# Todegal/HobbyRaytracer

Measured on AMD Instinct MI355X. Metric: Mrays/sec (path segments/s), teapot_scene.yaml 640x640 100spp, higher is better.
Workload: dtype f32

## Files before the change

hobbyraytracer_amd/csrc/hrt_hip.hip:

```cpp
#include <hip/hip_runtime.h>
#include <rccl/rccl.h>
#include <dlfcn.h>

#include <algorithm>
#include <cmath>
#include <cstdio>
#include <cstdlib>
#include <cstring>
#include <memory>
#include <new>
#include <string>
#include <thread>
#include <type_traits>
#include <vector>

#include "hrt_device.h"
#include "hrt_pack.h"
#include "hrt_roulette.h"
#include "hrt_aov.h"
#include "hrt_map.h"

using namespace hrt;

namespace {
// ... 1102 lines not shown
        local += weight(i);
        out[i + 1] = ok ? (float)((s_run[t] + local) / total) : 0.0f;
    }
    __syncthreads();
    if (t == 0) { out[0] = 0.0f; out[n] = 1.0f; }
    return total;
}
__global__ __launch_bounds__(256) void k_env_rows(const float* __restrict__ texels, int W, int H, int channels, float* __restrict__ cond,
                                                  double* __restrict__ row_total) {
    __shared__ double s_run[257];
    const int j = blockIdx.x;
    double phi0, dphi, c0, dc;
    env_cell_bounds<double>(0, j, W, H, phi0, dphi, c0, dc);
    const float* row = texels + (size_t)j * (size_t)W * (size_t)channels;
    const double total = env_block_cdf(W, [&](int i) { return env_texel_weight(row + (size_t)i * (size_t)channels, i, W, dc); },
                                       cond + (size_t)j * (size_t)(W + 1), s_run);
    if (threadIdx.x == 0) row_total[j] = total;
}
__global__ __launch_bounds__(256) void k_env_marginal(const double* __restrict__ row_total, int H, float* __restrict__ marg, double* __restrict__ total) {
    __shared__ double s_run[257];
    const double t = env_block_cdf(H, [&](int j) { return row_total[j]; }, marg, s_run);
    if (threadIdx.x == 0) total[0] = t;
}

#define HRT_TAIL_MAX_MESHES 4
struct TailMeshes { int n; int prim[HRT_TAIL_MAX_MESHES]; };
template <bool STATS, int DEPTH>
__global__ __launch_bounds__(256, DEPTH <= 24 ? 4 : 3) void k_wf_tail(DScene sc, hrt_params pr, RenderMap map, WfScene ws, TailMeshes tm, unsigned n_local, int s0, int round0,
                                                    int rounds_end, WfBuf w, DeviceCounters* counters, int leaf_num) {
    const unsigned lane = threadIdx.x & 63u;
    const unsigned wave = (blockIdx.x * blockDim.x + threadIdx.x) >> 6;
    const unsigned long long lt = (1ull << lane) - 1ull;
    __shared__ int s_stack[DEPTH * 256];
    constexpr uint32_t TABLE_BYTES = DEPTH <= 20 ? 4096 : (DEPTH <= 24 ? 1536 : 4096);
    __shared__ __attribute__((aligned(16))) uint32_t s_tables[TABLE_BYTES / 4];
    __shared__ float s_missq[4][7 * HRT_MISSQ_CAP];
    stage_tables(sc, s_tables, TABLE_BYTES);
    MissQueue mq;
    mq.f = s_missq[threadIdx.x >> 6]; mq.slot = (unsigned*)(mq.f + 6 * HRT_MISSQ_CAP); mq.count = 0;
    unsigned n_seg = 0, n_culled = 0;
    PathCounters pc; pc.rays = 0; pc.samples = 0; pc.mesh_hits = 0; pc.env_lookups = 0; pc.bvh.box_tests = 0; pc.bvh.tri_tests = 0;
    DCounters cnt; cnt.box_tests = 0; cnt.tri_tests = 0;
    HRT_FOR_MY_TASKS(task, w, wave, lane) {
        unsigned live = HRT_UNIFORM(w.live[task]), qn = HRT_UNIFORM(w.qn[task]), rn = HRT_UNIFORM(w.rn[task]);
        for (int r = round0; r < rounds_end && live; ++r) {
            const int par = r & 1;
            for (int m = 0; m < tm.n; ++m) {
                if (m > 0) {
                    qn = wf_pre_task<STATS>(sc, pr, map, n_local, s0, r, par, tm.prim[m - 1] + 1, tm.prim[m], w, task, live, lane, lt, n_culled, rn);
                    __builtin_amdgcn_fence(__ATOMIC_ACQ_REL, "workgroup");
                }
                if (rn) {
                    wf_ref_task<STATS>(wf_ref_mesh(sc, tm.prim[m], pr.quirks), pr, tm.prim[m], par, w, task, rn, s_stack + (threadIdx.x & ~63u), DEPTH * 64u, lane, cnt);
                    __builtin_amdgcn_fence(__ATOMIC_ACQ_REL, "workgroup");
                }
                if (qn) {
                    const ExtMesh em = wf_ext_mesh(sc, tm.prim[m], pr.quirks);
                    bool given = false;
                    const unsigned first0 = task * w.T, end0 = first0 + qn;
                    wf_ext_run<STATS>(em, pr, tm.prim[m], par, w, s_stack + threadIdx.x, lane, lt, leaf_num, cnt, [&](unsigned& first, unsigned& end) {
                        if (given) return false;
                        given = true; first = first0; end = end0;
                        return true;
                    });
                    __builtin_amdgcn_fence(__ATOMIC_ACQ_REL, "workgroup");
                }
            }
            wf_shade_task<STATS>(sc, pr, map, ws, n_local, s0, r, w, task, live, lane, lt, mq, pc, n_seg, n_culled, live, qn, rn);
            __builtin_amdgcn_fence(__ATOMIC_ACQ_REL, "workgroup");
        }
        if (lane == 0) { w.live[task] = live; w.qn[task] = qn; w.rn[task] = rn; }
    }
    if (mq.count) missq_flush<STATS>(sc, w, mq, lane, mq.count, pc);
    wf_shade_counters<STATS>(w, counters, wave, lane, n_seg, n_culled, pc);
    if (STATS) {
        const unsigned bt = wave_sum(cnt.box_tests), tt = wave_sum(cnt.tri_tests);
        if (lane == 0) {
            if (bt) atomicAdd(&counters->box_tests, (unsigned long long)bt);
            if (tt) atomicAdd(&counters->tri_tests, (unsigned long long)tt);
        }
    }
}

__device__ inline float4 wf_sample_value(const float4* __restrict__ rad, const float4* __restrict__ direct, size_t i, bool nee) {
    float4 r = rad[i];
    if (nee) { const float4 d = direct[i]; r.x = r.x + d.x; r.y = r.y + d.y; r.z = r.z + d.z; }
    return r;
}
__device__ inline void wf_fold_shadow(DeviceCounters* counters, unsigned long long* __restrict__ wave_shadow, unsigned n_wave_rays) {
    __shared__ unsigned long long total_s;
    if (threadIdx.x == 0) total_s = 0;
    __syncthreads();
    unsigned long long mine = 0;
    for (unsigned i = threadIdx.x; i < n_wave_rays; i += blockDim.x) { mine += wave_shadow[i]; wave_shadow[i] = 0; }
    if (mine) atomicAdd(&total_s, mine);
    __syncthreads();
    if (threadIdx.x == 0 && total_s) atomicAdd(&counters->shadow_rays, total_s);
}
template <bool NEE>
__global__ __launch_bounds__(256) void k_wf_reduce(const float4* __restrict__ rad, unsigned n_local, int chunk, int first_chunk, int last_chunk,
                                                   int spp, float* __restrict__ out, DeviceCounters* counters,
                                                   unsigned long long* __restrict__ wave_rays, unsigned n_wave_rays,
                                                   const float4* __restrict__ direct, unsigned long long* __restrict__ wave_shadow) {
    const unsigned stride = gridDim.x * blockDim.x;
    for (unsigned lp = blockIdx.x * blockDim.x + threadIdx.x; lp < n_local; lp += stride) {
        vec3 sum(0.0f);
        if (!first_chunk) sum = vec3(out[3ull * lp], out[3ull * lp + 1], out[3ull * lp + 2]);
        for (int s = 0; s < chunk; ++s) {
            const float4 r = wf_sample_value(rad, direct, (size_t)s * n_local + lp, NEE);
            sum += vec3(r.x, r.y, r.z);
        }
        if (last_chunk) sum = sum / static_cast<float>(spp);
        out[3ull * lp] = sum.x; out[3ull * lp + 1] = sum.y; out[3ull * lp + 2] = sum.z;
    }
    if (blockIdx.x == 0) {
        __shared__ unsigned long long total;
        if (threadIdx.x == 0) total = 0;
        __syncthreads();
        unsigned long long mine = 0;
        for (unsigned i = threadIdx.x; i < n_wave_rays; i += blockDim.x) { mine += wave_rays[i]; wave_rays[i] = 0; }
        if (mine) atomicAdd(&total, mine);
        __syncthreads();
        if (threadIdx.x == 0) {
            if (total) atomicAdd(&counters->rays, total);
            atomicAdd(&counters->samples, (unsigned long long)n_local * (unsigned long long)chunk);
        }
        if (NEE) wf_fold_shadow(counters, wave_shadow, n_wave_rays);
    }
}

__global__ __launch_bounds__(256) void k_wf_progress(const unsigned* __restrict__ live, unsigned n_tasks, unsigned long long base_plus_slots,
                                                     volatile unsigned long long* host_ctr) {
    __shared__ unsigned long long total;
    if (threadIdx.x == 0) total = 0;
    __syncthreads();
    unsigned long long mine = 0;
    for (unsigned i = threadIdx.x; i < n_tasks; i += blockDim.x) mine += live[i];
    if (mine) atomicAdd(&total, mine);
    __syncthreads();
    if (threadIdx.x == 0) { *host_ctr = base_plus_slots - total; __threadfence_system(); }
}
__global__ void k_set_progress(unsigned long long v, volatile unsigned long long* host_ctr) { *host_ctr = v; __threadfence_system(); }

__global__ __launch_bounds__(256) void k_unstripe(const float* __restrict__ gathered, float* __restrict__ film, int H, int W3, int R, int G, long long share) {
    const long long n = (long long)H * W3;
    for (long long i = (long long)blockIdx.x * blockDim.x + threadIdx.x; i < n; i += (long long)gridDim.x * blockDim.x) {
        const int row = (int)(i / W3), x = (int)(i - (long long)row * W3);
        const int b = row / R, g = b % G, local = (b / G) * R + (row - b * R);
        film[i] = gathered[(long long)g * share + (long long)local * W3 + x];
    }
}
__global__ __launch_bounds__(256) void k_restripe(const float* __restrict__ film, float* __restrict__ mine, int H, int W3, int R, int G, int rank, int rows) {
    const long long n = (long long)rows * W3;
    for (long long i = (long long)blockIdx.x * blockDim.x + threadIdx.x; i < n; i += (long long)gridDim.x * blockDim.x) {
        const int local = (int)(i / W3), x = (int)(i - (long long)local * W3);
        const int b = local / R, row = (b * G + rank) * R + (local - b * R);
        mine[i] = film[(long long)row * W3 + x];
    }
}
__global__ __launch_bounds__(256) void k_preview_mean(const float* __restrict__ sums, float* __restrict__ mean, long long n, float samples_done) {
    for (long long i = (long long)blockIdx.x * blockDim.x + threadIdx.x; i < n; i += (long long)gridDim.x * blockDim.x) mean[i] = sums[i] / samples_done;
}



__device__ inline float ad_luma(float r, float g, float b) { return 0.2126f * r + 0.7152f * g + 0.0722f * b; }
// ... 85 lines not shown
        const unsigned v = i < n ? blocks[i] : 0u;
        part[threadIdx.x] = v;
        __syncthreads();
        for (unsigned off = 1; off < 256; off <<= 1) {
            const unsigned t = threadIdx.x >= off ? part[threadIdx.x - off] : 0u;
            __syncthreads();
            part[threadIdx.x] += t;
            __syncthreads();
        }
        if (i < n) blocks[i] = carry + part[threadIdx.x] - v;
        carry += part[255];
        __syncthreads();
    }
    if (threadIdx.x == 0) blocks[n] = carry;
}
__global__ __launch_bounds__(256) void k_ad_mean(const float* __restrict__ sums, const int32_t* __restrict__ count, long long n,
                                                 float* __restrict__ mean) {
    for (long long i = (long long)blockIdx.x * blockDim.x + threadIdx.x; i < n; i += (long long)gridDim.x * blockDim.x) {
        const float c = static_cast<float>(count[i]);
        mean[3 * i] = sums[3 * i] / c; mean[3 * i + 1] = sums[3 * i + 1] / c; mean[3 * i + 2] = sums[3 * i + 2] / c;
    }
}

}

namespace {
thread_local std::string g_err;

hrt_status fail_hip(hipError_t e, const char* what) {
    g_err = std::string(what) + ": " + hipGetErrorString(e);
    return HRT_ERR_HIP;
}
hrt_status fail(hrt_status s, const std::string& msg) { g_err = msg; return s; }
}
extern "C" __attribute__((visibility("hidden"))) void hrt_set_last_error(const char* msg) { g_err = msg; }
namespace {

#define HIPCHK(expr)                                         \
    do {                                                     \
        hipError_t _e = (expr);                              \
        if (_e != hipSuccess) return fail_hip(_e, #expr);    \
    } while (0)
#define HRTCHK(expr)                                         \
    do {                                                     \
        hrt_status _s = (expr);                              \
        if (_s != HRT_OK) return _s;                         \
    } while (0)

class DevBuf {
public:
    DevBuf() = default;
    DevBuf(DevBuf&& o) noexcept : p_(o.p_) { o.p_ = nullptr; }
    DevBuf& operator=(DevBuf&& o) noexcept { if (this != &o) { reset(); p_ = o.p_; o.p_ = nullptr; } return *this; }
    DevBuf(const DevBuf&) = delete;
    DevBuf& operator=(const DevBuf&) = delete;
    ~DevBuf() { reset(); }
    hrt_status alloc(size_t bytes, const char* what) {
        reset();
        hipError_t e = hipMalloc(&p_, bytes);
        if (e == hipSuccess) return HRT_OK;
        p_ = nullptr;
        return fail(e == hipErrorOutOfMemory ? HRT_ERR_OOM : HRT_ERR_HIP, std::string(what) + ": " + hipGetErrorString(e));
    }
    void reset() { if (p_) (void)hipFree(p_); p_ = nullptr; }
    template <typename T = void> T* get() const { return static_cast<T*>(p_); }
    explicit operator bool() const { return p_ != nullptr; }
private:
    void* p_ = nullptr;
};

hrt_status upload(DevBuf& buf, const void* src, size_t bytes) {
    HRTCHK(buf.alloc(bytes ? bytes : 16, "hipMalloc"));
    if (bytes) HIPCHK(hipMemcpy(buf.get(), src, bytes, hipMemcpyHostToDevice));
    return HRT_OK;
}

bool finite3(const float* p) { return p[0] == p[0] && p[1] == p[1] && p[2] == p[2]; }
}

struct WfWorkspace {
    DevBuf base;
    size_t bytes = 0;
    size_t slots = 0;
    int depth = 0, n_mesh = 0;
    bool nee = false;
    bool lobes = false;
    WfBuf buf{};
};

struct hrt_scene {
    int device = 0;
    int n_cus = 256;
    DScene ds{};
    std::vector<DevBuf> allocs;
    std::vector<int> mesh_prims;
    std::vector<int> mesh_depths;
    int n_prims = 0;
    DeviceCounters* d_counters = nullptr;
    unsigned* d_work = nullptr;
    WfWorkspace wf;
    struct Pending { hipEvent_t a, b; };
    std::vector<Pending> pending, pending_trav;
    std::vector<hipEvent_t> event_pool;
    double kernel_ms = 0.0, traversal_ms = 0.0;
    uint64_t launches = 0, traversal_launches = 0;
    volatile unsigned long long* h_progress = nullptr;
    unsigned long long* d_progress = nullptr;
    unsigned long long progress_base = 0;
    volatile unsigned long long progress_total = 0;
    DevBuf ad_pix, ad_blocks;
    size_t ad_cap = 0;
    float4* d_lights = nullptr;
    int32_t* d_light_of = nullptr;
    int n_lights = 0;
    DevBuf env_marg, env_cond;
    int env_w = 0, env_h = 0;
    DevBuf emit_rec, emit_shade, emit_alias, emit_base;
    int n_emit = 0;
    int32_t rr_first = HRT_ROULETTE_FIRST_BOUNCE;
    float rr_floor = HRT_ROULETTE_Q_FLOOR;
};

namespace {

hrt_status validate(const hrt_flat_scene* f) {
    if (!f) return fail(HRT_ERR_INVALID, "flat scene is NULL");
    if (f->n_prims && !f->prims) return fail(HRT_ERR_INVALID, "prims is NULL");
    if (f->n_textures == 0 || !f->textures) return fail(HRT_ERR_INVALID, "scene needs at least the background texture");
    if (f->background_tex < 0 || (uint32_t)f->background_tex >= f->n_textures) return fail(HRT_ERR_INVALID, "background_tex out of range");
    for (uint32_t i = 0; i < f->n_textures; ++i) {
        const hrt_texture& t = f->textures[i];
        if (t.kind < HRT_TEX_SOLID || t.kind > HRT_TEX_ENV) return fail(HRT_ERR_INVALID, "texture kind out of range");
        if (t.kind == HRT_TEX_CHECKER) {
            if (t.even < 0 || (uint32_t)t.even >= f->n_textures || t.odd < 0 || (uint32_t)t.odd >= f->n_textures)
                return fail(HRT_ERR_INVALID, "checker child out of range");
        }
        if (t.kind == HRT_TEX_IMAGE || t.kind == HRT_TEX_ENV) {
            if (t.width < 0 || t.height < 0) return fail(HRT_ERR_INVALID, "negative texture size");
            if (t.width > 0 && t.height > 0) {
                const bool env = t.kind == HRT_TEX_ENV;
                if (env && t.channels < 3) return fail(HRT_ERR_INVALID, "environment map needs >= 3 channels");
                const uint64_t have = env ? f->n_texels_f32 : f->n_texels_u8;
                const uint64_t per = (uint64_t)t.width * (uint64_t)t.height;
                const uint64_t ch = env ? (uint64_t)t.channels : 3u;
                if (t.offset > have || per > (have - t.offset) / ch) return fail(HRT_ERR_INVALID, env ? "env texels out of range" : "image texels out of range");
                if (have && !(env ? (const void*)f->texels_f32 : (const void*)f->texels_u8)) return fail(HRT_ERR_INVALID, "texel array is NULL");
            }
        }
    }
    for (uint32_t i = 0; i < f->n_textures; ++i) {
        if (f->textures[i].kind != HRT_TEX_CHECKER) continue;
        std::vector<std::pair<uint32_t, int>> st;
        st.push_back({i, 1});
        while (!st.empty()) {
            auto [t, depth] = st.back(); st.pop_back();
            if (f->textures[t].kind != HRT_TEX_CHECKER) continue;
            if (depth > 4) return fail(HRT_ERR_UNSUPPORTED, "checkered textures nested more than 4 deep (or cyclic)");
            st.push_back({(uint32_t)f->textures[t].even, depth + 1});
            st.push_back({(uint32_t)f->textures[t].odd, depth + 1});
        }
    }
    if (f->n_materials && !f->materials) return fail(HRT_ERR_INVALID, "materials is NULL");
    if (f->n_meshes && !f->meshes) return fail(HRT_ERR_INVALID, "meshes is NULL");
    if (f->n_nodes && !f->nodes) return fail(HRT_ERR_INVALID, "nodes is NULL");
    auto tex_ok = [&](int32_t t) { return t < 0 || (uint32_t)t < f->n_textures; };
    for (uint32_t i = 0; i < f->n_materials; ++i) {
        const hrt_material& m = f->materials[i];
// ... 139 lines not shown
    if ((int64_t)p->width * p->height > (int64_t)1 << 30) return fail(HRT_ERR_UNSUPPORTED, "film larger than 2^30 pixels");
    if (((int64_t)p->width + 7) / 8 * (((int64_t)p->height + 7) / 8) * 64 > (int64_t)0x7fffffff) return fail(HRT_ERR_UNSUPPORTED, "film too thin: its 8x8-tile padding exceeds 2^31 pixels");
    if (p->samples < 1) return fail(HRT_ERR_INVALID, "samples must be >= 1");
    if (p->max_depth < 1) return fail(HRT_ERR_INVALID, "max_depth must be >= 1");
    if (p->max_depth > 65536) return fail(HRT_ERR_UNSUPPORTED, "max_depth above 65536 (the reference's is 50, main.cpp:32)");
    if (!(p->t_min == p->t_min)) return fail(HRT_ERR_INVALID, "t_min is NaN");
    if ((p->flags & HRT_FLAG_NEE_ENV) && !(p->flags & HRT_FLAG_NEE)) return fail(HRT_ERR_INVALID, "HRT_FLAG_NEE_ENV needs HRT_FLAG_NEE");
    if ((p->flags & HRT_FLAG_NEE_EMITTERS) && !(p->flags & HRT_FLAG_NEE)) return fail(HRT_ERR_INVALID, "HRT_FLAG_NEE_EMITTERS needs HRT_FLAG_NEE");
    if ((p->flags & HRT_FLAG_NEE_LOBES) && !(p->flags & HRT_FLAG_NEE)) return fail(HRT_ERR_INVALID, "HRT_FLAG_NEE_LOBES needs HRT_FLAG_NEE");
    if ((p->flags & HRT_FLAG_MEGAKERNEL) && (p->flags & HRT_FLAG_NEE)) return fail(HRT_ERR_UNSUPPORTED, "next-event estimation renders on the wavefront pipeline only");
    if ((p->flags & HRT_FLAG_MEGAKERNEL) && (p->flags & HRT_FLAG_STRATIFIED)) return fail(HRT_ERR_UNSUPPORTED, "the stratified sampler renders on the wavefront pipeline only");
    if ((p->flags & HRT_FLAG_MEGAKERNEL) && (p->flags & HRT_FLAG_ROULETTE)) return fail(HRT_ERR_UNSUPPORTED, "Russian roulette renders on the wavefront pipeline only");
    if ((p->flags & HRT_FLAG_STATS) && (p->flags & HRT_FLAG_ROULETTE)) return fail(HRT_ERR_UNSUPPORTED, "HRT_FLAG_ROULETTE has no counting kernels (HRT_FLAG_STATS); rays and shadow_rays are counted without them");
    return HRT_OK;
}

hrt_status env_table_device(const float* d_texels, int W, int H, int channels, float* d_marg, float* d_cond, bool* has) {
    DevBuf d_rows, d_total;
    HRTCHK(d_rows.alloc((size_t)H * sizeof(double), "hipMalloc(env table)"));
    HRTCHK(d_total.alloc(sizeof(double), "hipMalloc(env table)"));
    hipLaunchKernelGGL(k_env_rows, dim3((unsigned)H), dim3(256), 0, 0, d_texels, W, H, channels, d_cond, d_rows.get<double>());
    hipLaunchKernelGGL(k_env_marginal, dim3(1), dim3(256), 0, 0, d_rows.get<const double>(), H, d_marg, d_total.get<double>());
    HIPCHK(hipGetLastError());
    double total = 0.0;
    HIPCHK(hipMemcpy(&total, d_total.get(), sizeof(double), hipMemcpyDeviceToHost));
    *has = total > 0.0 && std::isfinite(total);
    return HRT_OK;
}

hrt_status check_stripes(int32_t R, int32_t rank, int32_t G) {
    if (R <= 0 || G <= 0 || rank < 0 || rank >= G) return fail(HRT_ERR_INVALID, "bad stripe partition");
    return HRT_OK;
}

int grid_for(const hrt_scene* sc, long long n) { return (int)std::min<long long>((n + 255) / 256, (long long)sc->n_cus * 8); }

template <typename F>
void with_bool(bool b, F&& f) {
    if (b) f(std::true_type{});
    else f(std::false_type{});
}

int depth_variant(int depth) { return depth <= 20 ? 20 : (depth <= 24 ? 24 : 32); }
template <typename F>
void with_depth(int variant, F&& f) {
    switch (variant) {
        case 20: f(std::integral_constant<int, 20>{}); break;
        case 24: f(std::integral_constant<int, 24>{}); break;
        default: f(std::integral_constant<int, 32>{}); break;
    }
}

hrt_status get_event(hrt_scene* sc, hipEvent_t* ev) {
    if (!sc->event_pool.empty()) { *ev = sc->event_pool.back(); sc->event_pool.pop_back(); return HRT_OK; }
    HIPCHK(hipEventCreate(ev));
    return HRT_OK;
}

hrt_status launch_megakernel(hrt_scene* sc, const hrt_camera* cam, const hrt_params* pr, const RenderMap& map, float* d_out,
                             hipStream_t stream) {
    HIPCHK(hipMemsetAsync(sc->d_work, 0, sizeof(unsigned), stream));
    const int blocks = grid_for(sc, map.total_items);
    with_bool(pr->flags & HRT_FLAG_STATS, [&](auto S) {
        hipLaunchKernelGGL(k_pathtrace<decltype(S)::value>, dim3(blocks), dim3(HRT_BLOCK), 0, stream, sc->ds, *cam, *pr, map, d_out, sc->d_counters, sc->d_work);
    });
    HIPCHK(hipGetLastError());
    return HRT_OK;
}

size_t wf_max_slots(const hrt_scene* sc, bool nee = false, bool lobes = false) {
    if (const char* e = getenv("HRT_WF_MAX_SLOTS")) { long long v = atoll(e); if (v > 0) return (size_t)v; }
    size_t cap = (size_t)48 << 20;
    size_t free_b = 0, total_b = 0;
    if (hipMemGetInfo(&free_b, &total_b) == hipSuccess) {
        free_b += sc->wf.bytes;
        cap = std::max(cap, (size_t)((double)free_b * 0.6 / (lobes ? 264.0 : (nee ? 232.0 : 184.0))));
    }
    return std::min(cap, (size_t)1 << 31);
}

size_t wf_counter_words(int depth, int n_mesh) { return (size_t)256 * (2 + (size_t)depth * (2 * (size_t)std::max(1, n_mesh) + 2)); }
size_t wf_ref_counter_words(int depth, int n_mesh) { return (size_t)512 * ((size_t)depth * (size_t)std::max(1, n_mesh) + 1); }

hrt_status wf_reserve(hrt_scene* sc, size_t slots, int depth, bool nee, bool lobes) {
    WfWorkspace& w = sc->wf;
    const int n_mesh = (int)sc->mesh_prims.size();
    if (w.base && w.slots >= slots && w.depth >= depth && w.n_mesh == n_mesh && (w.nee || !nee) && (w.lobes || !lobes)) return HRT_OK;
    if (w.base) { HIPCHK(hipDeviceSynchronize()); w = WfWorkspace(); }
    const size_t max_tasks = slots / 64 + 1;
    auto al = [](size_t x) { return (x + 255) & ~(size_t)255; };
    const size_t f4 = al((slots + 4096) * sizeof(float4));
    const size_t i4 = al((slots + 4096) * sizeof(int));
    const size_t ctr_words = wf_counter_words(depth, n_mesh) + wf_ref_counter_words(depth, n_mesh);
    const size_t ref_cap = max_tasks / HRT_REF_GROUPS + 1;
    const size_t total = (sc->ds.stale_ff ? 12 : 11) * f4 + 2 * i4 + 3 * al(max_tasks * sizeof(unsigned)) + al(ctr_words * sizeof(unsigned)) + al(ref_cap * HRT_REF_GROUPS * sizeof(uint2)) +
                         al((size_t)sc->n_cus * 32 * sizeof(unsigned long long)) +
                         (nee ? 3 * f4 + al((size_t)sc->n_cus * 32 * sizeof(unsigned long long)) : 0) +
                         (lobes ? 2 * f4 : 0);
    DevBuf base;
    HRTCHK(base.alloc(total, "hipMalloc(wavefront workspace)"));
    char* p = base.get<char>();
    auto take = [&](size_t bytes) { char* q = p; p += bytes; return q; };
    for (int k = 0; k < 2; ++k) {
        w.buf.S0[k] = (float4*)take(f4); w.buf.S1[k] = (float4*)take(f4); w.buf.S2[k] = (float4*)take(f4); w.buf.S3[k] = (float*)take(i4);
    }
    w.buf.E0 = (float4*)take(f4); w.buf.E1 = (float4*)take(f4); w.buf.E2 = (float4*)take(f4); w.buf.E3 = (float4*)take(f4);
    w.buf.rad = (float4*)take(f4);
    w.buf.S4 = sc->ds.stale_ff ? (float4*)take(f4) : nullptr;
    w.buf.live = (unsigned*)take(al(max_tasks * sizeof(unsigned)));
    w.buf.qn = (unsigned*)take(al(max_tasks * sizeof(unsigned)));
    w.buf.rn = (unsigned*)take(al(max_tasks * sizeof(unsigned)));
    w.buf.task_ctr = (unsigned*)take(al(ctr_words * sizeof(unsigned)));
    w.buf.ref_list = (uint2*)take(al(ref_cap * HRT_REF_GROUPS * sizeof(uint2)));
    w.buf.ref_cap = (unsigned)ref_cap;
    w.buf.n_wave_rays = (unsigned)sc->n_cus * 8u * 4u;
    w.buf.wave_rays = (unsigned long long*)take(al((size_t)w.buf.n_wave_rays * sizeof(unsigned long long)));
    HIPCHK(hipMemset(w.buf.wave_rays, 0, (size_t)w.buf.n_wave_rays * sizeof(unsigned long long)));
    if (nee) {
        w.buf.N[0] = (float4*)take((lobes ? 2 : 1) * f4); w.buf.N[1] = (float4*)take((lobes ? 2 : 1) * f4); w.buf.direct = (float4*)take(f4);
        w.buf.wave_shadow = (unsigned long long*)take(al((size_t)w.buf.n_wave_rays * sizeof(unsigned long long)));
        HIPCHK(hipMemset(w.buf.wave_shadow, 0, (size_t)w.buf.n_wave_rays * sizeof(unsigned long long)));
    }
    w.base = std::move(base); w.bytes = total; w.slots = slots; w.depth = depth; w.n_mesh = n_mesh; w.nee = nee; w.lobes = lobes;
    return HRT_OK;
}

hrt_status launch_wavefront(hrt_scene* sc, const hrt_camera* cam, const hrt_params* pr, const RenderMap& map, float* d_out,
                            hipStream_t stream, int s_first, int s_count, float* d_sq, int32_t* d_count) {
    const unsigned n_local = map_pixels(map);
    const int D = pr->max_depth;
    const int n_mesh = (int)sc->mesh_prims.size();
    const bool env = (pr->flags & HRT_FLAG_NEE) != 0 && (pr->flags & HRT_FLAG_NEE_ENV) != 0 && sc->env_marg;
    const bool emit = (pr->flags & HRT_FLAG_NEE) != 0 && (pr->flags & HRT_FLAG_NEE_EMITTERS) != 0 && sc->n_emit > 0;
    const bool nee = (pr->flags & HRT_FLAG_NEE) != 0 && (sc->n_lights > 0 || env || emit);
    const bool lobes = nee && (pr->flags & HRT_FLAG_NEE_LOBES) != 0;
    const bool strat = (pr->flags & HRT_FLAG_STRATIFIED) != 0;
    const bool rr = (pr->flags & HRT_FLAG_ROULETTE) != 0;
    size_t cap = wf_max_slots(sc, nee, lobes);
    const int s_end = s_first + s_count;
    int chunk = (int)std::min<size_t>((size_t)s_count, std::max<size_t>(1, cap / n_local));
    hrt_status st;
    for (;;) {
        const size_t slots = (size_t)n_local * chunk;
        if (slots >= ((size_t)1 << 32) - 4096) return fail(HRT_ERR_UNSUPPORTED, "tile too large for 32-bit slot ids");
        st = wf_reserve(sc, slots, D, nee, lobes);
        if (st != HRT_ERR_OOM || chunk == 1) break;
        chunk = (chunk + 1) / 2;
    }
    if (st != HRT_OK) return st;
    WfBuf w = sc->wf.buf;
    if (nee) { w.lights = sc->d_lights; w.light_of = sc->d_light_of; w.n_lights = sc->n_lights; }
    if (env) { w.env_marg = sc->env_marg.get<float>(); w.env_cond = sc->env_cond.get<float>(); w.env_w = sc->env_w; w.env_h = sc->env_h; }
    if (emit) {
        w.emit_rec = sc->emit_rec.get<const float4>(); w.emit_shade = sc->emit_shade.get<const float4>();
        w.emit_alias = sc->emit_alias.get<const float2>(); w.emit_base = sc->emit_base.get<const int32_t>(); w.n_emit = sc->n_emit;
    }
    WfScene ws;
    ws.has_mesh = n_mesh > 0;
    ws.first_mesh = n_mesh > 0 ? sc->mesh_prims.front() : sc->n_prims;
    ws.rest = n_mesh > 0 ? sc->mesh_prims.back() + 1 : sc->n_prims;
    const bool stats = (pr->flags & HRT_FLAG_STATS) != 0, timing = (pr->flags & HRT_FLAG_TIMING) != 0;
    const bool progress = (pr->flags & HRT_FLAG_PROGRESS) != 0 && sc->d_progress;
    int ext_per_cu_env = 0;
    if (const char* e = getenv("HRT_EXT_BLOCKS_PER_CU")) ext_per_cu_env = std::min(10, std::max(1, atoi(e)));
    const size_t batch_slots = (size_t)n_local * (size_t)chunk;
    int tail_round = batch_slots <= ((size_t)512 << 10) ? 1 : (batch_slots <= ((size_t)6 << 20) ? 8 : (batch_slots <= ((size_t)12 << 20) ? 24 : D));
    if (const char* e = getenv("HRT_WF_TAIL_ROUND")) tail_round = std::max(1, atoi(e));
    if (n_mesh > HRT_TAIL_MAX_MESHES) tail_round = D;
    const bool stale_ff = sc->ds.stale_ff && (pr->quirks & HRT_Q3_TRI_NO_FACE);
    if (stale_ff) tail_round = D;
    if (nee) tail_round = D;
    if (strat) tail_round = D;
    if (rr) tail_round = D;
    tail_round = std::min(tail_round, D);
    int leaf_num = 48;
    if (const char* e = getenv("HRT_EXT_LEAF_NUM")) leaf_num = atoi(e);
    leaf_num = std::min(64, std::max(1, leaf_num));

    for (int s0 = s_first; s0 < s_end; s0 += chunk) {
        const int c = std::min(chunk, s_end - s0);
        const unsigned n_slots = n_local * (unsigned)c;
        auto round64 = [](size_t x) { return (x + 63) & ~(size_t)63; };
        const size_t t_large = round64(n_slots / ((size_t)sc->n_cus * 64));
        const size_t t_small = std::min<size_t>(1280, std::max<size_t>(256, round64(n_slots / ((size_t)sc->n_cus * 16))));
        size_t T = std::min<size_t>(4096, std::max(t_large, t_small));
        if (const char* e = getenv("HRT_WF_TASK_SIZE")) T = std::min<size_t>(4096, std::max<size_t>(64, round64((size_t)atoi(e))));
        w.T = (unsigned)T;
        w.n_tasks = (unsigned)((n_slots + T - 1) / T);
        const int task_blocks = (int)std::min<size_t>(((size_t)w.n_tasks + 3) / 4, (size_t)sc->n_cus * 8);
        unsigned task_groups = HRT_TASK_GROUPS;
        {
            const double P = (double)n_local / (double)T;
            auto covers = [&](unsigned G) {
                double worst = 1e30;
                for (int m = 1; m <= 4; ++m) {
                    const double r = std::fmod(m * P, (double)G), d = std::min(r, (double)G - r);
                    worst = std::min(worst, d * (double)c / (m * P));
                }
                return worst;
            };
            if (P > 1.0 && c > 1 && covers(HRT_TASK_GROUPS) < 1.0) {
                double best = -1.0;
                for (unsigned G : {251u, 241u, 239u, 233u, 229u, 227u, 223u, 211u, 199u, 197u, 193u, 191u}) {
                    const double v = covers(G);
                    if (v >= 1.0) { task_groups = G; break; }
                    if (v > best) { best = v; task_groups = G; }
                }
            }
            if (const char* e = getenv("HRT_WF_TASK_GROUPS")) task_groups = (unsigned)std::min(256, std::max(1, atoi(e)));
        }
        unsigned* const ctr_base = sc->wf.buf.task_ctr;
        HIPCHK(hipMemsetAsync(ctr_base, 0, (wf_counter_words(D, n_mesh) + wf_ref_counter_words(D, n_mesh)) * sizeof(unsigned), stream));
        unsigned* const ref_base = ctr_base + wf_counter_words(D, n_mesh);
        const int nm1 = std::max(1, n_mesh);
        auto ref_block = [&](int r, int m) { return ref_base + 512 * (size_t)((r < D && m < nm1) ? r * nm1 + m : D * nm1); };
        size_t launch_no = 0;
        const bool force_dynamic = getenv("HRT_WF_DYNAMIC_TASKS") != nullptr;
        auto next_counters = [&](unsigned waves) {
            w.task_ctr = ctr_base + 256 * launch_no++;
            w.n_groups = std::min<unsigned>(task_groups, waves);
            w.pull_k = (w.n_tasks <= waves && !force_dynamic) ? 0u : std::min(32u, std::max(1u, w.n_tasks / (waves * 4u)));
            w.group_q = w.n_tasks / w.n_groups; w.group_r = w.n_tasks % w.n_groups;
        };
        if (nee) HIPCHK(hipMemsetAsync(w.direct, 0, (size_t)n_slots * sizeof(float4), stream));
        next_counters((unsigned)task_blocks * 4u);
        w.ref_prod = ref_block(0, 0); w.ref_cons = ref_block(D, 0);
        with_bool(stats, [&](auto S) {
            hipLaunchKernelGGL(strat ? k_wf_gen_st<decltype(S)::value> : k_wf_gen<decltype(S)::value>, dim3(task_blocks), dim3(256), 0, stream, sc->ds, *cam, *pr, map, ws, n_local, s0, n_slots, w, sc->d_counters);
        });
        for (int r = 0; r < tail_round; ++r) {
            const int par = r & 1;
            for (int m = 0; m < n_mesh; ++m) {
                const int mp = sc->mesh_prims[m];
                if (m > 0) {
                    const int p0 = sc->mesh_prims[m - 1] + 1;
                    next_counters((unsigned)task_blocks * 4u);
                    w.ref_prod = ref_block(r, m); w.ref_cons = ref_block(D, 0);
                    with_bool(stats, [&](auto S) {
                        hipLaunchKernelGGL(k_wf_pre<decltype(S)::value>, dim3(task_blocks), dim3(256), 0, stream, sc->ds, *pr, map, n_local, s0, r, par, p0, mp, w, sc->d_counters);
                    });
                }
                hipEvent_t ea = nullptr, eb = nullptr;
                if (timing) { HRTCHK(get_event(sc, &ea)); HRTCHK(get_event(sc, &eb)); HIPCHK(hipEventRecord(ea, stream)); }
                const int variant = depth_variant(sc->mesh_depths[m]);
                const int ext_blocks = sc->n_cus * (ext_per_cu_env ? ext_per_cu_env : (variant == 32 ? 4 : 6));
                next_counters((unsigned)ext_blocks * (HRT_BLOCK / 64));
                w.ref_prod = ref_block(D, 0); w.ref_cons = ref_block(r, m);
                with_bool(stats, [&](auto S) { with_depth(variant, [&](auto DP) {
                    hipLaunchKernelGGL((k_wf_ext<decltype(S)::value, decltype(DP)::value>), dim3(ext_blocks), dim3(HRT_BLOCK), 0, stream, sc->ds, *pr, mp, par, w,
                                       sc->d_counters, leaf_num);
                }); });
                if (timing) { HIPCHK(hipEventRecord(eb, stream)); sc->pending_trav.push_back({ea, eb}); }
            }
            if (stale_ff) {
                next_counters((unsigned)task_blocks * 4u);
                hipLaunchKernelGGL(k_wf_stale, dim3(task_blocks), dim3(256), 0, stream, sc->ds, *pr, par, w);
            }
            next_counters((unsigned)task_blocks * 4u);
            w.ref_prod = ref_block(r + 1, 0); w.ref_cons = ref_block(D, 0);
            if (rr) {
                auto shade_rr = [&](auto kernel) {
                    hipLaunchKernelGGL(kernel, dim3(task_blocks), dim3(256), 0, stream, sc->ds, *pr, map, ws, n_local, s0, r, w, sc->d_counters, (int)sc->rr_first, sc->rr_floor);
                };
                if (lobes)
                    with_bool(env, [&](auto E) { with_bool(emit, [&](auto M) {
                        shade_rr(strat ? k_wf_shade_st_rr<false, true, decltype(E)::value, decltype(M)::value, true> : k_wf_shade_rr<false, true, decltype(E)::value, decltype(M)::value, true>);
                    }); });
                else if (emit)
                    with_bool(env, [&](auto E) { shade_rr(strat ? k_wf_shade_st_rr<false, true, decltype(E)::value, true> : k_wf_shade_rr<false, true, decltype(E)::value, true>); });
                else if (env)
                    shade_rr(strat ? k_wf_shade_st_rr<false, true, true> : k_wf_shade_rr<false, true, true>);
                else
                    with_bool(nee, [&](auto N) { shade_rr(strat ? k_wf_shade_st_rr<false, decltype(N)::value> : k_wf_shade_rr<false, decltype(N)::value>); });
            } else if (lobes) {
                with_bool(env, [&](auto E) { with_bool(emit, [&](auto M) { with_bool(stats, [&](auto S) {
                    hipLaunchKernelGGL((strat ? k_wf_shade_st<decltype(S)::value, true, decltype(E)::value, decltype(M)::value, true> : k_wf_shade<decltype(S)::value, true, decltype(E)::value, decltype(M)::value, true>), dim3(task_blocks), dim3(256), 0, stream, sc->ds, *pr,
                                       map, ws, n_local, s0, r, w, sc->d_counters);
                }); }); });
            } else if (emit) {
                with_bool(env, [&](auto E) { with_bool(stats, [&](auto S) {
                    hipLaunchKernelGGL((strat ? k_wf_shade_st<decltype(S)::value, true, decltype(E)::value, true> : k_wf_shade<decltype(S)::value, true, decltype(E)::value, true>), dim3(task_blocks), dim3(256), 0, stream, sc->ds, *pr, map, ws,
                                       n_local, s0, r, w, sc->d_counters);
                }); });
            } else if (env) {
                with_bool(stats, [&](auto S) {
                    hipLaunchKernelGGL((strat ? k_wf_shade_st<decltype(S)::value, true, true> : k_wf_shade<decltype(S)::value, true, true>), dim3(task_blocks), dim3(256), 0, stream, sc->ds, *pr, map, ws, n_local, s0, r, w,
                                       sc->d_counters);
                });
            } else {
                with_bool(nee, [&](auto N) { with_bool(stats, [&](auto S) {
                    hipLaunchKernelGGL((strat ? k_wf_shade_st<decltype(S)::value, decltype(N)::value> : k_wf_shade<decltype(S)::value, decltype(N)::value>), dim3(task_blocks), dim3(256), 0, stream, sc->ds, *pr, map, ws, n_local, s0, r, w,
                                       sc->d_counters);
                }); });
            }
            if (nee && r + 1 < D) {
                next_counters((unsigned)task_blocks * 4u);
                if (lobes)
                    with_bool(env, [&](auto E) { with_bool(emit, [&](auto M) {
                        hipLaunchKernelGGL((strat ? k_wf_shadow_st<decltype(E)::value, decltype(M)::value, true> : k_wf_shadow<decltype(E)::value, decltype(M)::value, true>), dim3(task_blocks), dim3(HRT_BLOCK), 0, stream, sc->ds, *pr, map, n_local, s0, r, w);
                    }); });
                else if (emit)
                    hipLaunchKernelGGL((strat ? (env ? k_wf_shadow_st<true, true> : k_wf_shadow_st<false, true>) : (env ? k_wf_shadow<true, true> : k_wf_shadow<false, true>)),
                                       dim3(task_blocks), dim3(HRT_BLOCK), 0, stream, sc->ds, *pr, map, n_local, s0, r, w);
                else
                    hipLaunchKernelGGL((strat ? (env ? k_wf_shadow_st<true> : k_wf_shadow_st<false>) : (env ? k_wf_shadow<true> : k_wf_shadow<false>)),
                                       dim3(task_blocks), dim3(HRT_BLOCK), 0, stream, sc->ds, *pr, map, n_local, s0, r, w);
            }
            if (progress)
                hipLaunchKernelGGL(k_wf_progress, dim3(1), dim3(256), 0, stream, w.live, w.n_tasks, sc->progress_base + n_slots, sc->d_progress);
        }
        if (tail_round < D) {
            TailMeshes tm{};
            tm.n = n_mesh;
            int need = 0;
            for (int m = 0; m < n_mesh; ++m) { tm.prim[m] = sc->mesh_prims[m]; need = std::max(need, sc->mesh_depths[m]); }
            const int variant = depth_variant(need);
            const int tail_blocks = (int)std::min<size_t>(((size_t)w.n_tasks + 3) / 4, (size_t)sc->n_cus * (variant == 32 ? 3 : 4));
            next_counters((unsigned)tail_blocks * 4u);
            w.ref_prod = ref_block(D, 0); w.ref_cons = ref_block(D, 0);
            with_bool(stats, [&](auto S) { with_depth(variant, [&](auto DP) {
                hipLaunchKernelGGL((k_wf_tail<decltype(S)::value, decltype(DP)::value>), dim3(tail_blocks), dim3(256), 0, stream, sc->ds, *pr, map, ws, tm, n_local, s0,
                                   tail_round, D, w, sc->d_counters, leaf_num);
            }); });
        }
        const int rblocks = grid_for(sc, n_local);
        if (map.mode == 2)
            hipLaunchKernelGGL(nee ? k_wf_reduce_list<true> : k_wf_reduce_list<false>, dim3(rblocks), dim3(256), 0, stream, w.rad, map.pix, n_local, c, s0 == 0 ? 1 : 0, s0 + c, d_out, d_sq, d_count,
                               sc->d_counters, w.wave_rays, w.n_wave_rays, (const float4*)w.direct, w.wave_shadow);
        else
            hipLaunchKernelGGL(nee ? k_wf_reduce<true> : k_wf_reduce<false>, dim3(rblocks), dim3(256), 0, stream, w.rad, n_local, c, s0 == 0 ? 1 : 0, s0 + c >= pr->samples ? 1 : 0, pr->samples, d_out,
                               sc->d_counters, w.wave_rays, w.n_wave_rays, (const float4*)w.direct, w.wave_shadow);
        if (progress) {
            sc->progress_base += n_slots;
            hipLaunchKernelGGL(k_set_progress, dim3(1), dim3(1), 0, stream, sc->progress_base, sc->d_progress);
        }
        HIPCHK(hipGetLastError());
    }
    return HRT_OK;
}

hrt_status launch_pathtrace(hrt_scene* sc, const hrt_camera* cam, const hrt_params* pr, const RenderMap& map, float* d_out,
                            hipStream_t stream, int s_first = 0, int s_count = -1, float* d_sq = nullptr, int32_t* d_count = nullptr) {
    if (map.total_items <= 0) return HRT_OK;
    if (s_count < 0) s_count = pr->samples - s_first;
    if (s_first < 0 || s_count < 1 || s_first + s_count > pr->samples) return fail(HRT_ERR_INVALID, "sample range outside [0, samples)");
    if ((pr->flags & HRT_FLAG_MEGAKERNEL) && (s_first != 0 || s_count != pr->samples))
        return fail(HRT_ERR_UNSUPPORTED, "the megakernel path renders all samples in one launch (no partial sample ranges)");
    if (pr->flags & HRT_FLAG_PROGRESS) {
        hipLaunchKernelGGL(k_set_progress, dim3(1), dim3(1), 0, stream, 0ull, sc->d_progress);
        sc->progress_base = 0;
        sc->progress_total = (unsigned long long)map_pixels(map) * (unsigned long long)s_count;
    }
    hipEvent_t a, b;
    HRTCHK(get_event(sc, &a));
    HRTCHK(get_event(sc, &b));
    HIPCHK(hipEventRecord(a, stream));
    HRTCHK((pr->flags & HRT_FLAG_MEGAKERNEL) ? launch_megakernel(sc, cam, pr, map, d_out, stream)
                                             : launch_wavefront(sc, cam, pr, map, d_out, stream, s_first, s_count, d_sq, d_count));
    if (pr->flags & HRT_FLAG_PROGRESS) {
        hipLaunchKernelGGL(k_set_progress, dim3(1), dim3(1), 0, stream, (unsigned long long)sc->progress_total, sc->d_progress);
        HIPCHK(hipGetLastError());
    }
    HIPCHK(hipEventRecord(b, stream));
    sc->pending.push_back({a, b});
    sc->launches++;
    return HRT_OK;
}

hrt_status fold_events(hrt_scene* sc, std::vector<hrt_scene::Pending>& list, double& ms_sum, uint64_t* n) {
    for (auto& p : list) {
        HIPCHK(hipEventSynchronize(p.b));
        float ms = 0.0f;
        HIPCHK(hipEventElapsedTime(&ms, p.a, p.b));
        ms_sum += ms;
        if (n) ++*n;
        sc->event_pool.push_back(p.a); sc->event_pool.push_back(p.b);
    }
    list.clear();
    return HRT_OK;
}
hrt_status fold_pending(hrt_scene* sc) {
    HRTCHK(fold_events(sc, sc->pending, sc->kernel_ms, nullptr));
    return fold_events(sc, sc->pending_trav, sc->traversal_ms, &sc->traversal_launches);
}

struct HostArray { void* host; size_t bytes; };

template <size_t N, typename Run>
hrt_status render_via_host(hrt_scene* sc, hrt_stats* stats, const HostArray (&arrays)[N], bool copy_in, const char* what, Run run) {
    HIPCHK(hipSetDevice(sc->device));
    hrt_stats now;
    HRTCHK(hrt_scene_stats(sc, &now));
    size_t total = 0;
    for (const HostArray& a : arrays) total += a.bytes;
    if (total) {
        DevBuf buf;
        HRTCHK(buf.alloc(total, "hipMalloc"));
        void* dev[N];
        for (size_t k = 0, at = 0; k < N; at += arrays[k++].bytes) dev[k] = buf.get<char>() + at;
        auto copy = [&](bool in) {
            for (size_t k = 0; k < N; ++k) {
                const hipError_t e = in ? hipMemcpy(dev[k], arrays[k].host, arrays[k].bytes, hipMemcpyHostToDevice)
                                        : hipMemcpy(arrays[k].host, dev[k], arrays[k].bytes, hipMemcpyDeviceToHost);
                if (e != hipSuccess) return fail_hip(e, (std::string(in ? "hipMemcpy H2D " : "hipMemcpy D2H ") + what).c_str());
            }
// ... 954 lines not shown
```

Measured before the change: 6660.

## Compact live paths into merged tasks before persistent tail kernel

Adds a merge kernel that, at a chosen bounce round, compacts the surviving path state of K adjacent wavefront tasks into one larger task. The tail kernel then runs over fewer, fuller tasks. The goal is to balance load and cut per-task overhead when many tasks hold few live rays in late bounces. In exchange it adds a compaction pass with extra memory traffic, extra slack buffers and per-task counters. It only applies under narrow conditions: single mesh, no NEE, no stratification, no roulette, and a large batch.

```diff
diff --git a/hobbyraytracer_amd/csrc/hrt_hip.hip b/hobbyraytracer_amd/csrc/hrt_hip.hip
--- a/hobbyraytracer_amd/csrc/hrt_hip.hip
+++ b/hobbyraytracer_amd/csrc/hrt_hip.hip
@@ -1208,6 +1208,11 @@
     }
 }
 
+#define HRT_MERGE_TASKS_PER_WAVE 1
+extern "C" __attribute__((visibility("hidden"))) void hrt_wf_merge_launch(float4* s0, float4* s1, float4* s2, float* s3, const unsigned* live, unsigned T,
+                                                                          unsigned n_tasks, unsigned K, unsigned* live_m, unsigned* qn_m, unsigned* rn_m,
+                                                                          hipStream_t stream);
+
 __device__ inline float4 wf_sample_value(const float4* __restrict__ rad, const float4* __restrict__ direct, size_t i, bool nee) {
     float4 r = rad[i];
     if (nee) { const float4 d = direct[i]; r.x = r.x + d.x; r.y = r.y + d.y; r.z = r.z + d.z; }
@@ -1459,7 +1464,9 @@
     DevBuf base;
     size_t bytes = 0;
     size_t slots = 0;
+    size_t slack = 0;
     int depth = 0, n_mesh = 0;
+    unsigned *live_m = nullptr, *qn_m = nullptr, *rn_m = nullptr;
     bool nee = false;
     bool lobes = false;
     WfBuf buf{};
@@ -1765,18 +1772,18 @@
 size_t wf_counter_words(int depth, int n_mesh) { return (size_t)256 * (2 + (size_t)depth * (2 * (size_t)std::max(1, n_mesh) + 2)); }
 size_t wf_ref_counter_words(int depth, int n_mesh) { return (size_t)512 * ((size_t)depth * (size_t)std::max(1, n_mesh) + 1); }
 
-hrt_status wf_reserve(hrt_scene* sc, size_t slots, int depth, bool nee, bool lobes) {
+hrt_status wf_reserve(hrt_scene* sc, size_t slots, size_t slack, int depth, bool nee, bool lobes) {
     WfWorkspace& w = sc->wf;
     const int n_mesh = (int)sc->mesh_prims.size();
-    if (w.base && w.slots >= slots && w.depth >= depth && w.n_mesh == n_mesh && (w.nee || !nee) && (w.lobes || !lobes)) return HRT_OK;
+    if (w.base && w.slots >= slots && w.slack >= slack && w.depth >= depth && w.n_mesh == n_mesh && (w.nee || !nee) && (w.lobes || !lobes)) return HRT_OK;
     if (w.base) { HIPCHK(hipDeviceSynchronize()); w = WfWorkspace(); }
     const size_t max_tasks = slots / 64 + 1;
     auto al = [](size_t x) { return (x + 255) & ~(size_t)255; };
-    const size_t f4 = al((slots + 4096) * sizeof(float4));
-    const size_t i4 = al((slots + 4096) * sizeof(int));
+    const size_t f4 = al((slots + slack) * sizeof(float4));
+    const size_t i4 = al((slots + slack) * sizeof(int));
     const size_t ctr_words = wf_counter_words(depth, n_mesh) + wf_ref_counter_words(depth, n_mesh);
     const size_t ref_cap = max_tasks / HRT_REF_GROUPS + 1;
-    const size_t total = (sc->ds.stale_ff ? 12 : 11) * f4 + 2 * i4 + 3 * al(max_tasks * sizeof(unsigned)) + al(ctr_words * sizeof(unsigned)) + al(ref_cap * HRT_REF_GROUPS * sizeof(uint2)) +
+    const size_t total = (sc->ds.stale_ff ? 12 : 11) * f4 + 2 * i4 + 6 * al(max_tasks * sizeof(unsigned)) + al(ctr_words * sizeof(unsigned)) + al(ref_cap * HRT_REF_GROUPS * sizeof(uint2)) +
                          al((size_t)sc->n_cus * 32 * sizeof(unsigned long long)) +
                          (nee ? 3 * f4 + al((size_t)sc->n_cus * 32 * sizeof(unsigned long long)) : 0) +
                          (lobes ? 2 * f4 : 0);
@@ -1793,6 +1800,9 @@
     w.buf.live = (unsigned*)take(al(max_tasks * sizeof(unsigned)));
     w.buf.qn = (unsigned*)take(al(max_tasks * sizeof(unsigned)));
     w.buf.rn = (unsigned*)take(al(max_tasks * sizeof(unsigned)));
+    unsigned* const live_m = (unsigned*)take(al(max_tasks * sizeof(unsigned)));
+    unsigned* const qn_m = (unsigned*)take(al(max_tasks * sizeof(unsigned)));
+    unsigned* const rn_m = (unsigned*)take(al(max_tasks * sizeof(unsigned)));
     w.buf.task_ctr = (unsigned*)take(al(ctr_words * sizeof(unsigned)));
     w.buf.ref_list = (uint2*)take(al(ref_cap * HRT_REF_GROUPS * sizeof(uint2)));
     w.buf.ref_cap = (unsigned)ref_cap;
@@ -1804,7 +1814,8 @@
         w.buf.wave_shadow = (unsigned long long*)take(al((size_t)w.buf.n_wave_rays * sizeof(unsigned long long)));
         HIPCHK(hipMemset(w.buf.wave_shadow, 0, (size_t)w.buf.n_wave_rays * sizeof(unsigned long long)));
     }
-    w.base = std::move(base); w.bytes = total; w.slots = slots; w.depth = depth; w.n_mesh = n_mesh; w.nee = nee; w.lobes = lobes;
+    w.live_m = live_m; w.qn_m = qn_m; w.rn_m = rn_m;
+    w.base = std::move(base); w.bytes = total; w.slots = slots; w.slack = slack; w.depth = depth; w.n_mesh = n_mesh; w.nee = nee; w.lobes = lobes;
     return HRT_OK;
 }
 
@@ -1822,11 +1833,55 @@
     size_t cap = wf_max_slots(sc, nee, lobes);
     const int s_end = s_first + s_count;
     int chunk = (int)std::min<size_t>((size_t)s_count, std::max<size_t>(1, cap / n_local));
+    auto round64 = [](size_t x) { return (x + 63) & ~(size_t)63; };
+    auto task_size = [&](size_t n_slots) {
+        const size_t t_large = round64(n_slots / ((size_t)sc->n_cus * 64));
+        const size_t t_small = std::min<size_t>(1280, std::max<size_t>(256, round64(n_slots / ((size_t)sc->n_cus * 16))));
+        size_t T = std::min<size_t>(4096, std::max(t_large, t_small));
+        if (const char* e = getenv("HRT_WF_TASK_SIZE")) T = std::min<size_t>(4096, std::max<size_t>(64, round64((size_t)atoi(e))));
+        return T;
+    };
+    TailMeshes tm{};
+    int tail_variant = 20;
+    if (n_mesh <= HRT_TAIL_MAX_MESHES) {
+        tm.n = n_mesh;
+        int need = 0;
+        for (int m = 0; m < n_mesh; ++m) { tm.prim[m] = sc->mesh_prims[m]; need = std::max(need, sc->mesh_depths[m]); }
+        tail_variant = depth_variant(need);
+    }
+    const size_t tail_blocks_max = (size_t)sc->n_cus * (tail_variant == 32 ? 3 : 4);
+    const bool stale_ff = sc->ds.stale_ff && (pr->quirks & HRT_Q3_TRI_NO_FACE);
+    int merge_forced = -1;
+    bool merge_off = false;
+    if (const char* e = getenv("HRT_WF_MERGE_ROUND")) {
+        if (!strcmp(e, "off")) merge_off = true;
+        else merge_forced = std::max(0, atoi(e));
+    }
+    size_t merge_factor = 0;
+    if (const char* e = getenv("HRT_WF_MERGE_FACTOR")) merge_factor = (size_t)std::max(0, atoi(e));
+    const bool merge_ok = !merge_off && !getenv("HRT_WF_TAIL_ROUND") && n_mesh <= 1 && !stale_ff && !nee && !strat && !rr;
+    struct MergePlan { unsigned k; int round; };
+    auto merge_plan = [&](size_t n_slots) {
+        const MergePlan none{1u, D};
+        if (!merge_ok) return none;
+        const size_t T = task_size(n_slots), n_tasks = (n_slots + T - 1) / T;
+        const size_t waves = tail_blocks_max * 4 * HRT_MERGE_TASKS_PER_WAVE;
+        const size_t k = std::min(n_tasks, merge_factor ? merge_factor : (n_tasks + waves - 1) / waves);
+        if (k < 2) return none;
+        if (merge_forced >= 0) return merge_forced < D ? MergePlan{(unsigned)k, merge_forced} : none;
+        const size_t n_merged = (n_tasks + k - 1) / k, M = k * T;
+        if (n_slots <= ((size_t)6 << 20) || n_merged * 8 < waves * 7 || M > 12288) return none;
+        const int round = M <= 3072 ? 16 : (M <= 6144 ? 24 : 28);
+        return round < D ? MergePlan{(unsigned)k, round} : none;
+    };
+    auto batch_slack = [&](size_t n_slots) { return std::max<size_t>(4096, (size_t)merge_plan(n_slots).k * task_size(n_slots)); };
     hrt_status st;
     for (;;) {
         const size_t slots = (size_t)n_local * chunk;
-        if (slots >= ((size_t)1 << 32) - 4096) return fail(HRT_ERR_UNSUPPORTED, "tile too large for 32-bit slot ids");
-        st = wf_reserve(sc, slots, D, nee, lobes);
+        size_t slack = batch_slack(slots);
+        if (s_count % chunk) slack = std::max(slack, batch_slack((size_t)n_local * (size_t)(s_count % chunk)));
+        if (slots >= ((size_t)1 << 32) - slack) return fail(HRT_ERR_UNSUPPORTED, "tile too large for 32-bit slot ids");
+        st = wf_reserve(sc, slots, slack, D, nee, lobes);
         if (st != HRT_ERR_OOM || chunk == 1) break;
         chunk = (chunk + 1) / 2;
     }
@@ -1850,7 +1905,6 @@
     int tail_round = batch_slots <= ((size_t)512 << 10) ? 1 : (batch_slots <= ((size_t)6 << 20) ? 8 : (batch_slots <= ((size_t)12 << 20) ? 24 : D));
     if (const char* e = getenv("HRT_WF_TAIL_ROUND")) tail_round = std::max(1, atoi(e));
     if (n_mesh > HRT_TAIL_MAX_MESHES) tail_round = D;
-    const bool stale_ff = sc->ds.stale_ff && (pr->quirks & HRT_Q3_TRI_NO_FACE);
     if (stale_ff) tail_round = D;
     if (nee) tail_round = D;
     if (strat) tail_round = D;
@@ -1863,13 +1917,15 @@
     for (int s0 = s_first; s0 < s_end; s0 += chunk) {
         const int c = std::min(chunk, s_end - s0);
         const unsigned n_slots = n_local * (unsigned)c;
-        auto round64 = [](size_t x) { return (x + 63) & ~(size_t)63; };
-        const size_t t_large = round64(n_slots / ((size_t)sc->n_cus * 64));
-        const size_t t_small = std::min<size_t>(1280, std::max<size_t>(256, round64(n_slots / ((size_t)sc->n_cus * 16))));
-        size_t T = std::min<size_t>(4096, std::max(t_large, t_small));
-        if (const char* e = getenv("HRT_WF_TASK_SIZE")) T = std::min<size_t>(4096, std::max<size_t>(64, round64((size_t)atoi(e))));
+        const size_t T = task_size(n_slots);
         w.T = (unsigned)T;
         w.n_tasks = (unsigned)((n_slots + T - 1) / T);
+        w.live = sc->wf.buf.live; w.qn = sc->wf.buf.qn; w.rn = sc->wf.buf.rn;
+        const MergePlan plan = merge_plan(n_slots);
+        const unsigned merge_by = plan.k;
+        const int merge_round = plan.round;
+        const bool merge = merge_by >= 2;
+        const int per_round_end = merge ? merge_round + 1 : tail_round;
         const int task_blocks = (int)std::min<size_t>(((size_t)w.n_tasks + 3) / 4, (size_t)sc->n_cus * 8);
         unsigned task_groups = HRT_TASK_GROUPS;
         {
@@ -1911,7 +1967,7 @@
         with_bool(stats, [&](auto S) {
             hipLaunchKernelGGL(strat ? k_wf_gen_st<decltype(S)::value> : k_wf_gen<decltype(S)::value>, dim3(task_blocks), dim3(256), 0, stream, sc->ds, *cam, *pr, map, ws, n_local, s0, n_slots, w, sc->d_counters);
         });
-        for (int r = 0; r < tail_round; ++r) {
+        for (int r = 0; r < per_round_end; ++r) {
             const int par = r & 1;
             for (int m = 0; m < n_mesh; ++m) {
                 const int mp = sc->mesh_prims[m];
@@ -1935,6 +1991,7 @@
                 }); });
                 if (timing) { HIPCHK(hipEventRecord(eb, stream)); sc->pending_trav.push_back({ea, eb}); }
             }
+            if (merge && r == merge_round) break;
             if (stale_ff) {
                 next_counters((unsigned)task_blocks * 4u);
                 hipLaunchKernelGGL(k_wf_stale, dim3(task_blocks), dim3(256), 0, stream, sc->ds, *pr, par, w);
@@ -1992,18 +2049,20 @@
             if (progress)
                 hipLaunchKernelGGL(k_wf_progress, dim3(1), dim3(256), 0, stream, w.live, w.n_tasks, sc->progress_base + n_slots, sc->d_progress);
         }
-        if (tail_round < D) {
-            TailMeshes tm{};
-            tm.n = n_mesh;
-            int need = 0;
-            for (int m = 0; m < n_mesh; ++m) { tm.prim[m] = sc->mesh_prims[m]; need = std::max(need, sc->mesh_depths[m]); }
-            const int variant = depth_variant(need);
-            const int tail_blocks = (int)std::min<size_t>(((size_t)w.n_tasks + 3) / 4, (size_t)sc->n_cus * (variant == 32 ? 3 : 4));
+        if (merge) {
+            const unsigned n_merged = (w.n_tasks + merge_by - 1) / merge_by;
+            const int mpar = merge_round & 1;
+            hrt_wf_merge_launch(w.S0[mpar], w.S1[mpar], w.S2[mpar], w.S3[mpar], w.live, w.T, w.n_tasks, merge_by, sc->wf.live_m, sc->wf.qn_m, sc->wf.rn_m, stream);
+            w.T *= merge_by; w.n_tasks = n_merged;
+            w.live = sc->wf.live_m; w.qn = sc->wf.qn_m; w.rn = sc->wf.rn_m;
+        }
+        if (merge || tail_round < D) {
+            const int tail_blocks = (int)std::min<size_t>(((size_t)w.n_tasks + 3) / 4, tail_blocks_max);
             next_counters((unsigned)tail_blocks * 4u);
             w.ref_prod = ref_block(D, 0); w.ref_cons = ref_block(D, 0);
-            with_bool(stats, [&](auto S) { with_depth(variant, [&](auto DP) {
+            with_bool(stats, [&](auto S) { with_depth(tail_variant, [&](auto DP) {
                 hipLaunchKernelGGL((k_wf_tail<decltype(S)::value, decltype(DP)::value>), dim3(tail_blocks), dim3(256), 0, stream, sc->ds, *pr, map, ws, tm, n_local, s0,
-                                   tail_round, D, w, sc->d_counters, leaf_num);
+                                   merge ? merge_round : tail_round, D, w, sc->d_counters, leaf_num);
             }); });
         }
         const int rblocks = grid_for(sc, n_local);
diff --git a/hobbyraytracer_amd/csrc/hrt_merge.hip b/hobbyraytracer_amd/csrc/hrt_merge.hip
--- /dev/null
+++ b/hobbyraytracer_amd/csrc/hrt_merge.hip
@@ -0,0 +1,37 @@
+#include <hip/hip_runtime.h>
+
+namespace {
+__device__ inline unsigned uniform(unsigned x) { return (unsigned)__builtin_amdgcn_readfirstlane((int)x); }
+
+__global__ __launch_bounds__(256) void k_wf_merge(float4* s0, float4* s1, float4* s2, float* s3, const unsigned* __restrict__ live, unsigned T, unsigned n_tasks,
+                                                  unsigned K, unsigned n_merged, unsigned* __restrict__ live_m, unsigned* __restrict__ qn_m, unsigned* __restrict__ rn_m) {
+    const unsigned lane = threadIdx.x & 63u;
+    const unsigned m = uniform((blockIdx.x * blockDim.x + threadIdx.x) >> 6);
+    if (m >= n_merged) return;
+    const unsigned first = m * K, last = first + K < n_tasks ? first + K : n_tasks;
+    const unsigned base = first * T;
+    unsigned total = 0;
+    for (unsigned t = first; t < last; ++t) {
+        const unsigned n = uniform(live[t]);
+        const unsigned src = t * T, dst = base + total;
+        if (dst != src) {
+            for (unsigned j0 = 0; j0 < n; j0 += 64) {
+                const bool mine = j0 + lane < n;
+                float4 a = make_float4(0, 0, 0, 0), b = a, c = a;
+                float az = 0.0f;
+                if (mine) { a = s0[src + j0 + lane]; b = s1[src + j0 + lane]; c = s2[src + j0 + lane]; az = s3[src + j0 + lane]; }
+                if (mine) { s0[dst + j0 + lane] = a; s1[dst + j0 + lane] = b; s2[dst + j0 + lane] = c; s3[dst + j0 + lane] = az; }
+            }
+        }
+        total += n;
+    }
+    if (lane == 0) { live_m[m] = total; qn_m[m] = 0; rn_m[m] = 0; }
+}
+}
+
+extern "C" __attribute__((visibility("hidden"))) void hrt_wf_merge_launch(float4* s0, float4* s1, float4* s2, float* s3, const unsigned* live, unsigned T,
+                                                                          unsigned n_tasks, unsigned K, unsigned* live_m, unsigned* qn_m, unsigned* rn_m,
+                                                                          hipStream_t stream) {
+    const unsigned n_merged = (n_tasks + K - 1) / K;
+    hipLaunchKernelGGL(k_wf_merge, dim3((n_merged + 3) / 4), dim3(256), 0, stream, s0, s1, s2, s3, live, T, n_tasks, K, n_merged, live_m, qn_m, rn_m);
+}
```

Measured after the change: 6850, median of 6. 2.9% higher.
